# CederGroupHub/smol

Measured on AMD Instinct MI355X. Metric: attempted MC flips/s (node) + ns/flip/replica, 4096-site FCC canonical, higher is better.
Workload: dtype f64

## Files before the change

smol_amd/csrc/engine.hip:

```cpp
#include <array>
#include <map>
#include <string>
#include <thread>

#include "smolmc_common.h"

thread_local std::string smolmc_g_err;

__device__ __forceinline__ double block_sum(double v, double *sh) {
    v = wave_sum(v);
    const int lane = threadIdx.x & 63, wave = threadIdx.x >> 6, nw = blockDim.x >> 6;
    __syncthreads();
    if (lane == 0) sh[wave] = v;
    __syncthreads();
    double s = 0;
    for (int i = 0; i < nw; ++i) s += sh[i];
    return s;
}

__global__ void __launch_bounds__(256) eval_full_kernel(const RefTables T, const uint8_t *occ_all,
                                                        double *out_all, const int ce_only, const int nocc, const int M) {
    __shared__ double sh[8];
    extern __shared__ __attribute__((aligned(16))) unsigned char eval_smem[];
    const int m_eff = M > 0 ? M : 1;
// ... 635 lines not shown
            S.feat = mode.lazy() ? 0u : (uint32_t)feat;
            S.live = mode.corr_kf ? (uint32_t)t->orb_nfunc[k.orbit] : 1u;
            S.w = folded ? scale : t->ce_coefs[feat] * scale;
            S.fs = scale;
            double dmax = 0.0;
            const double *D = L.dt.data() + doff_of[key];
            for (size_t z = 0; z < L.tlen; ++z) dmax = std::max(dmax, std::fabs(D[z]));
            sum_abs += std::fabs(S.w) * dmax;
        }
        sum_abs_max = std::max(sum_abs_max, sum_abs);
    }
    L.fast_eps = 2.0 * sum_abs_max * ldexp(1.0, -19);
    return L;
}

static int commit_lean_tables(smolmc_handle *h, const smolmc_tables *t, const SiteClasses &sc, const LeanMode &mode, int NSL, int MML,
                              const Swizzle &w, std::vector<uint16_t> &lidx, const LeanDeltaTables &L) {
    LeanParams &lp = h->lp;
    memset(&lp, 0, sizeof(LeanParams));
    lp.swz_a = w.a; lp.swz_m = w.m; lp.swz_b = w.b; lp.Nlds = w.Nlds;
    lp.fast_eps = L.fast_eps;
    lp.ktab8 = (uint32_t)L.tlen * 8u;
    lp.nt8 = (uint32_t)L.NTP * 8u;
    lp.snt8 = (uint32_t)L.NTP * 8u * (uint32_t)t->max_species;
    TRY(dev_upload(h, lidx.data(), lidx.size(), &lp.idx));
    h->lean_idx_host = std::move(lidx);
    TRY(dev_upload(h, L.dt.data(), L.dt.size(), &lp.dt));
    if (mode.corr_kf) TRY(dev_upload(h, L.dtk.data(), L.dtk.size(), &lp.dtk));
    TRY(dev_upload(h, L.ls.data(), L.ls.size(), &lp.slots));
    lp.dt_len = (int)L.dt.size();
    h->lean_kf = mode.corr_kf ? SMOLMC_LEAN_MAX_KF : 0;
    h->lazy_tables = mode.lazy();
    h->lean_tables = true;
    h->lean_nslot = NSL; h->lean_mm = MML; h->lean_ncls = (int)sc.class_rep.size();
    h->site_class_host = sc.site_class;
    return 0;
}

static int build_mc_tables(smolmc_handle *h, const smolmc_tables *t) {
    const GeneralLimits lim = general_limits(t, h->Npad);
    if (lim.error) return fail(lim.error);
    if (lim.universal) return no_general(h, lim.universal);
    const SiteClasses sc = site_classes(t, lim);
    if (sc.universal) return no_general(h, sc.universal);
// ... 379 lines not shown
static int create_impl(const smolmc_tables *t, const smolmc_config *cfg, smolmc_handle **out, std::vector<int32_t> *new_of);

extern "C" void *smolmc_debug_relabel(const smolmc_tables *t, int32_t *new_of_out) {
    if (!t || validate_tables(t)) return nullptr;
    std::vector<int32_t> new_of = plan_relabelling(t);
    if (new_of.empty()) return nullptr;
    std::vector<int32_t> old_of(new_of.size());
    for (size_t p = 0; p < new_of.size(); ++p) old_of[new_of[p]] = (int32_t)p;
    RelabelledTables *rt = new RelabelledTables();
    relabel_tables(t, new_of, old_of, *rt);
    if (new_of_out) std::copy(new_of.begin(), new_of.end(), new_of_out);
    return rt;
}
extern "C" void smolmc_debug_relabel_free(void *p) { delete (RelabelledTables *)p; }

extern "C" int smolmc_create(const smolmc_tables *t, const smolmc_config *cfg, smolmc_handle **out) {
    if (!t || !cfg || !out) return fail("null argument");
    if (cfg->n_replicas <= 0) return fail("n_replicas must be positive");
    if (int rc = validate_tables(t)) return rc;
    std::vector<int32_t> new_of = plan_relabelling(t);
    if (new_of.empty()) return create_impl(t, cfg, out, nullptr);
    std::vector<int32_t> old_of(new_of.size());
    for (size_t p = 0; p < new_of.size(); ++p) old_of[new_of[p]] = (int32_t)p;
    RelabelledTables rt;
    relabel_tables(t, new_of, old_of, rt);
    return create_impl(&rt.t, cfg, out, &new_of);
}

static int wl_sum_mode_of(const smolmc_handle *h) { return (h->cfg.wl_update_period == 1 && !smolmc_env(ENV_WL_RUNNING_MEAN)) ? 1 : 0; }
static int cu_count(const smolmc_handle *h) {
// ... 319 lines not shown
    lp.tf_n = t->n_flip_vectors;
    lp.tf_sw = t->swap_weight;
    lp.tf_ln_len = ln_len;
    return 0;
}

struct LeanPlan {
    bool take = false;
    bool late = false;
    int sbase = -1, nact = 0, nc = 0;
    std::vector<double> mu_row, bias_pair, qrow, dgrow;
    bool field = false;
    bool solo = false;
    int occ = 0, wpb = 4, tf_ln_len = 0;
    size_t lds = 0, lds8 = 0;
};
static LeanPlan decide_lean(const smolmc_handle *h, const smolmc_tables *t) {
    const smolmc_config *cfg = &h->cfg;
    const KParams &kp = h->kp;
    const LeanParams &lp = h->lp;
    const bool wl = is_wl(h), table = is_table(h);
    const int wl_sum_mode = wl_sum_mode_of(h), Fk = lean_features(h, t), brows = kp.bias_rows;
    LeanPlan p;
    const bool table_wl = wl && table;
    const bool lean = h->lean_tables && Fk <= 64 &&
                (!wl || ((wl_sum_mode || (table_wl && cfg->wl_update_period < (1ll << 31))) &&
                         h->F <= 63 && cfg->wl_check_period < (1ll << 31))) &&
                (!t->has_ewald || kp.ew_compact) && t->n_sublattices == 1 && h->lean_ncls == 1 &&
                h->lean_nslot <= 4 && !smolmc_env(ENV_FORCE_GENERAL);
    if (!lean) return p;
// ... 29 lines not shown
            p.field = true;
            p.lds = with_field;
        }
    }
    if (wl && t->has_ewald && !p.field) return p;
    p.take = true;
    if (!wl && !t->has_ewald && !t->bias_type && !h->lean_kf && !table && !smolmc_env(ENV_NO_SOLO)) {
        const size_t pw = ((size_t)lp.Nlds + 64 * 8 + 15) & ~(size_t)15;
        const size_t solo_lds = pw + ((size_t)lp.dt_len + 24) * 8;
        if (solo_lds * 16 <= 160 * 1024 - 16 * 256) {
            p.solo = true;
            p.lds = solo_lds;
            if ((long)cfg->n_replicas > 16L * cu_count(h) && solo_lds * 24 <= 160 * 1024 - 24 * 256 &&
                !smolmc_env(ENV_NO_OCC6))
                p.occ = 6;
        }
    }
    if (table) {
        p.lds += 48 * 8;
        const size_t half = 80 * 1024, with_ln = p.lds + (size_t)(nact + 1) * 8;
        if (with_ln <= 150 * 1024 && (with_ln <= half || p.lds > half)) {
            p.tf_ln_len = nact + 1;
            p.lds += (size_t)(nact + 1) * 8;
        }
        const size_t per_wave = (size_t)lp.Nlds + 64 * 8 + 64 + (p.field ? (size_t)kp.ew_nact * 8 : 0);
        const size_t lds8 = p.lds + 4 * per_wave;
        if (!wl && lds8 <= 160 * 1024 && p.lds > 40 * 1024 && cfg->n_replicas % 8 == 0 &&
            (long)cfg->n_replicas >= 8L * cu_count(h)) {
            p.wpb = 8;
            p.lds8 = lds8;
// ... 14 lines not shown
    for (double v : p.mu_row) mmax = std::max(mmax, std::fabs(v));
    h->fast_eps_plain = lp.fast_eps; h->fast_eps_widenings = 1; h->mu_max_create = mmax; h->d_mu_create = lp.mu_row;
    lean_set_fast_eps(h, mmax);
    lean_fill_state(h, t, lp, 64, is_table(h) ? kp.wl_sum_mode : 1);
    lp.sbase = p.sbase; lp.nact = p.nact; lp.ncodes = p.nc;
    if (t->has_ewald) { lp.ew_act = kp.ew_act; lp.ew_qs = kp.ew_qs; lp.ew_dg = kp.ew_dg; lp.ew_frozen = kp.ew_frozen; }
    lp.ew_field = 0;
    if (p.field) {
        if (dev_upload(h, p.qrow.data(), 8, &lp.ew_qrow) || dev_upload(h, p.dgrow.data(), 8, &lp.ew_dgrow)) return 1;
        lp.ew_phi = kp.ew_phi;
        lp.ew_field = 1;
    }
    if (p.solo) {
        std::vector<uint32_t> wide(h->lean_idx_host.begin(), h->lean_idx_host.end());
        if (dev_upload(h, wide.data(), wide.size(), &lp.idx32)) return 1;
    }
    if (is_table(h) && lean_fill_table(h, t, lp, p.nc, p.nact, p.tf_ln_len)) return 1;
    h->lean_lds = p.lds;
    h->lean_solo = p.solo;
    h->lean_occ = p.occ;
    h->lean_wpb = p.wpb;
    h->lean_lds_wpb8 = p.lds8;
    return 0;
}

struct LeanMultiPlan {
    bool take = false;
    std::string reason;
    int sbase[4], nact[4], ncodes[4], cls[4];
    double cum[4], mmax = 0.0;
    std::vector<double> mu_rows, q_rows, dg_rows, bias_pairs;
    int ndims = 0, max_nact = 0, wpb = 0;
    bool phi_lds = false;
    size_t lds = 0;
};
// ... 312 lines not shown
     {"lean-multi", nullptr, nullptr, L3(multi), L3(multi_replay), L3(multi_table_replay), L3(multi_wmu)},
     {"lean-multi", nullptr, nullptr, L3(multi_bias), L3(multi_bias_replay), NONE, L3(multi_bias_wmu)},
     {"lean-multi", " wl=multi", " wl=multi-mean", L3(multi_wl), L3(multi_wl_replay), NONE, NONE},
     {"lean-multi", " wl=multi", " wl=multi-mean", L3(multi_wl_kf), NONE, NONE, NONE},
     {"lean-multi", nullptr, nullptr, L3(multi_table_bias), NONE, NONE, L3(multi_table_bias_wmu)},
     {"lean-multi", " wl=multi", " wl=multi-mean", L3(multi_table_wl), NONE, NONE, NONE},
};
#undef L2
#undef L3
#undef NONE
static_assert(sizeof(lean_families) / sizeof(lean_families[0]) == K_MULTI_TABLE_WL - K_LEAN + 1, "one row per lean family");
static LeanLauncher lean_launcher(const smolmc_handle *h, bool replay) {
    const LeanFamilyRow &row = lean_families[h->family - K_LEAN];
    const int i = h->lean_nslot == 2 ? 0 : (h->lean_nslot == 4 ? 1 : 2);
    if (!replay && h->lp.mu_stride) return row.walker_mu[i];
    return !replay ? row.run[i] : (h->cfg.step_type == SMOLMC_STEP_TABLE_FLIP ? row.table_replay[i] : row.replay[i]);
}

static KernelFamily family_of(const smolmc_handle *h, const LeanPlan &one, const LeanMultiPlan &multi) {
    const bool wl = is_wl(h), table = is_table(h), bias = h->kp.bias_type != 0;
    if (one.take)
        return bias ? (table ? K_TABLE_BIAS : K_LEAN_BIAS) : (wl && table) ? K_TABLE_WL : h->lean_kf ? K_LEAN_CORR : wl ? K_WL : K_LEAN;
    if (multi.take)
        return wl ? (h->lean_kf ? K_MULTI_WL_KF : table ? K_MULTI_TABLE_WL : K_MULTI_WL)
                  : bias ? (table ? K_MULTI_TABLE_BIAS : K_MULTI_BIAS) : K_MULTI;
    return (table || !h->general_ok) ? K_UNIVERSAL : K_GENERAL;
}

static int create_impl(const smolmc_tables *t, const smolmc_config *cfg, smolmc_handle **out, std::vector<int32_t> *new_of) {
    if (t->max_species > 255) return fail("more than 255 species codes per site");
// ... 388 lines not shown

extern "C" int smolmc_sync(smolmc_handle *h) {
    if (!h) return fail("null handle");
    HIPCHK(hipSetDevice(h->device));
    HIPCHK(hipStreamSynchronize(h->stream));
    return 0;
}

extern "C" int smolmc_kernel_info(const smolmc_handle *h, char *buf, int n) {
    if (!h || !buf || n <= 0) return fail("null argument");
    if (h->dist) return smolmc_dist_kernel_info(h, buf, n);
    const LeanFamilyRow *row = h->lean() ? &lean_families[h->family - K_LEAN] : nullptr;
    if (h->univ())
        snprintf(buf, (size_t)n, "universal occ=%s field=%d lds=%zu (%s)", h->up.occ_lds ? "lds" : "hbm", h->kp.ew_field,
                 (size_t)h->up.lds_shared + (size_t)h->up.lds_per_wave * h->univ_wpb, h->general_ok ? "TableFlip outside the lean families" : h->general_reason.c_str());
    else if (row)
        snprintf(buf, (size_t)n, "%s nslot=%d mm=%d field=%d lds=%zu%s", row->name,
                 h->lean_nslot, h->lean_mm, h->lp.ew_field, h->lean_lds,
                 h->lean_solo ? (h->lean_occ ? " solo=1 occ=6" : " solo=1") : (h->lean_kf ? " kf=1" : ""));
    else
        snprintf(buf, (size_t)n, "general nslot=%d mm=%d field=%d lds=%zu", h->nslot, h->mm, h->kp.ew_field,
                 h->lds_bytes);
    {
        const size_t used = strlen(buf);
        const bool gx = row && h->lp.ew_field && h->lp.ew_gx && used + 40 < (size_t)n;
        if (gx)
            snprintf(buf + used, (size_t)n - used, " gx=%dx%dx%dx%d", h->ew_gx_blocks, h->ew_gx_dims[0], h->ew_gx_dims[1],
                     h->ew_gx_dims[2]);
        const char *wl_tag = !row || (gx && h->family == K_WL) ? nullptr : (h->lp.wl.sum_mode ? row->wl_sums : row->wl_means);
        if (wl_tag && strlen(buf) + 24 < (size_t)n) strncat(buf, wl_tag, (size_t)n - strlen(buf) - 1);
        if (is_lazy(h) && strlen(buf) + 16 < (size_t)n) strncat(buf, " lazy-features", (size_t)n - strlen(buf) - 1);
        if (h->relabelled && strlen(buf) + 16 < (size_t)n) strncat(buf, " relabelled=1", (size_t)n - strlen(buf) - 1);
        if (!h->walker_mu.empty() && strlen(buf) + 48 < (size_t)n)
            snprintf(buf + strlen(buf), (size_t)n - strlen(buf), " walker_mu=1 mu_max=%.17g", h->mu_max);
// ... 807 lines not shown
```

smol_amd/csrc/mc_lean.h:

```cpp
#pragma once
#include "smolmc_common.h"

template <int CTRL> __device__ __forceinline__ double dpp_xor_add(double v) {
    const int lo = __builtin_amdgcn_update_dpp(__double2loint(v), __double2loint(v), CTRL, 0xf, 0xf, true);
    const int hi = __builtin_amdgcn_update_dpp(__double2hiint(v), __double2hiint(v), CTRL, 0xf, 0xf, true);
    return v + __hiloint2double(hi, lo);
}
__device__ __forceinline__ double wave_sum_all(double v) {
    v = dpp_xor_add<0xB1>(v);
    v = dpp_xor_add<0x4E>(v);
    v = dpp_xor_add<0x141>(v);
    v = dpp_xor_add<0x140>(v);
    {
        const unsigned lo = (unsigned)__double2loint(v), hi = (unsigned)__double2hiint(v);
        const auto a = __builtin_amdgcn_permlane16_swap(lo, lo, false, false);
        const auto b = __builtin_amdgcn_permlane16_swap(hi, hi, false, false);
        v = __hiloint2double((int)b[0], (int)a[0]) + __hiloint2double((int)b[1], (int)a[1]);
    }
    {
        const unsigned lo = (unsigned)__double2loint(v), hi = (unsigned)__double2hiint(v);
        const auto a = __builtin_amdgcn_permlane32_swap(lo, lo, false, false);
        const auto b = __builtin_amdgcn_permlane32_swap(hi, hi, false, false);
        v = __hiloint2double((int)b[0], (int)a[0]) + __hiloint2double((int)b[1], (int)a[1]);
    }
// ... 249 lines not shown
#define SMOLMC_LDS_F64(a) (*(const double *)(uintptr_t)(a))
#endif
template <bool ABS> __device__ __forceinline__ uint8_t occ_ld(const uint8_t *occ, uint32_t a) {
    if constexpr (ABS) return SMOLMC_LDS_U8(a);
    else return occ[a];
}
__device__ __forceinline__ uint32_t opaque_u32(uint32_t v) {
    asm volatile("" : "+s"(v));
    return v;
}
template <bool ABS> __device__ __forceinline__ void occ_st(uint8_t *occ, uint32_t a, uint8_t v) {
    if constexpr (ABS) SMOLMC_LDS_U8(a) = v;
    else occ[a] = v;
}

template <int NSLOT, int MM, int STEP, bool HAS_MU, int EWX, bool WL, bool BIAS = false, bool SOLO = false,
          int KF = 0, int OCC = 0, bool REPLAY = false>
__global__ void __attribute__((amdgpu_waves_per_eu(OCC ? OCC : 1, OCC ? OCC : 8)))
__launch_bounds__(256) mc_lean_kernel(const LeanParams P) {
    static_assert(KF == 0 || (!WL && !BIAS && !SOLO), "correlation-function tables: plain Metropolis layouts only");
    static_assert(!REPLAY || (!WL && OCC == 0), "replay: Metropolis variants (Wang-Landau: mc_wl_kernel)");
    constexpr int NACC = KF ? KF : 1;
    constexpr int EWM = EWX & 3;
    constexpr bool WMU = (EWX & 4) != 0;
    static_assert(!WMU || (HAS_MU && !WL && !REPLAY), "per-walker chemical potentials: semigrand Metropolis variants");
    constexpr bool HAS_EW = EWM != 0, ew_field = EWM == 2;
    extern __shared__ __attribute__((aligned(16))) unsigned char smem[];
    if ((uint32_t)(uintptr_t)smem != 0u) __builtin_trap();
    const int lane = threadIdx.x & 63;
    const int wave = SOLO ? 0 : threadIdx.x >> 6;
    const int nwaves = SOLO ? 1 : blockDim.x >> 6;
    const int r = uni(blockIdx.x * nwaves + wave);
    const size_t per_wave = (size_t)P.Nlds + 64 * 8 + (WL ? (size_t)P.wl.L * 24 : 0) +
                            ((HAS_EW && ew_field) ? 64 + (size_t)P.ew_nact * 8 : 0);
    double *s_dt = SOLO ? (double *)(smem + ((per_wave + 15) & ~(size_t)15)) : (double *)smem;
    const uint32_t dt_off = SOLO ? (uint32_t)((per_wave + 15) & ~(size_t)15) : 0u;
    double *s_mu = s_dt + P.dt_len;
    double *s_q = s_mu + 8, *s_dg = s_mu + 16;
    unsigned char *wbase = SOLO ? smem : (unsigned char *)(s_mu + 24) + (size_t)wave * per_wave;
    uint8_t *occ = wbase;
// ... 32 lines not shown
    if (!live) return;

    constexpr bool EPRE = HAS_EW && STEP == SMOLMC_STEP_FLIP && !REPLAY;
    uint32_t ereg[27] = {};
    bool epre_on = false;
    if (EPRE) {
        const LeanParamsKernarg Q = rare_params();
        const uint32_t *E8 = Q->ew_E8;
        epre_on = ew_field && Q->ew_gx != nullptr && (Q->ew_nact >> 6) >= 27;
        if (epre_on) {
#pragma unroll
            for (int u = 0; u < 27; ++u) ereg[u] = E8[64 * u + lane];
        }
    }

    uint32_t doff8[NSLOT], st8[NSLOT][MM], sfeat[NSLOT];
    double wgt[NSLOT], acc[NSLOT], sfs[NSLOT];
    double accK[NSLOT][NACC];
    uint32_t kslot[NSLOT];
#pragma unroll
    for (int it = 0; it < NSLOT; ++it) {
        const LeanSlot sl = P.slots[it * 64 + lane];
        doff8[it] = sl.doff8 + dt_off;
        sfeat[it] = sl.feat;
        sfs[it] = sl.live ? sl.fs : 0.0;
        kslot[it] = sl.live;
#pragma unroll
        for (int m = 0; m < MM; ++m) st8[it][m] = sl.stride8[m];
        wgt[it] = sl.w;
        acc[it] = 0.0;
#pragma unroll
        for (int k = 0; k < NACC; ++k) accK[it][k] = 0.0;
    }
    const int wl_stride = WL ? P.F : 64;
    const int wl_k = WL ? max(1, min(8, 63 / max(wl_stride, 1))) : 1;
    uint32_t sfeat_wl[NSLOT];
#pragma unroll
    for (int it = 0; it < NSLOT; ++it) sfeat_wl[it] = sfeat[it] + (uint32_t)((lane % wl_k) * wl_stride);
    int wl_rd[8];
#pragma unroll
    for (int k = 0; k < 8; ++k) wl_rd[k] = (WL && k < wl_k && lane < wl_stride) ? lane + k * wl_stride : 63;
    auto wl_cur_feat = [&]() -> double {
        const int f = lane < wl_stride ? lane : 0;
// ... 39 lines not shown
    constexpr bool FAST = !WL && !HAS_EW;
    float thr_lo = 0.0f, thr_hi = 0.0f;
    const double inv_nbeta = FAST ? 1.0 / nbeta : 0.0;
    uint32_t nacc_before = 0;
    int nsite = 0, naddr = 0;
    double *featp = P.features + (size_t)r * P.F;
    const double base_feat = lane < P.F ? featp[lane] : 0.0;
    uint32_t smp_countdown = P.smp.every ? (uint32_t)P.smp.every : 0xffffffffu;
    long long smp_index = 0;
    uint32_t W0 = 0;
    int cand[4] = {0, 0, 0, 0}, canda[4] = {0, 0, 0, 0};
    double vGc = 0.0;
    double logu = 0.0;
    unsigned long long batch64_base = ~0ull;
    unsigned long long batch_base = ~0ull;
    constexpr int ROW = NSLOT * MM;
    constexpr int NW = SOLO ? ROW : ROW / 2;
    constexpr uint32_t ENT = SOLO ? 4u : 2u;
    constexpr uint32_t SITE_BYTES = 64u * ROW * ENT;
    const __amdgpu_buffer_rsrc_t idx_rs = __builtin_amdgcn_make_buffer_rsrc(
        SOLO ? (void *)P.idx32 : (void *)P.idx, 0, 0x7fffffff, 0x00020000);
    const uint32_t lane_voff = (uint32_t)lane * (ROW * ENT);

    int s1, a1;
    RowWords<NW> row1;
    uint32_t ridx = 0;
    double lu_rp = 0.0;
    int rp_bad = 0;
    auto rp_site = [&](const uint32_t i) -> int {
        const int v = uni(P.rp_steps[((size_t)r * (uint32_t)P.steps + i) * 4]);
        return v >= 0 ? v : sbase;
    };
    {
        if (REPLAY) {
            s1 = rp_site(0u);
        } else {
            const unsigned long long sp = step - 1ull;
            const uint32_t w = (uint32_t)uni((int)philox4x32_10((uint32_t)sp, (uint32_t)(sp >> 32), 0u, 0u,
                                                                key0, key1).w[1]);
            s1 = sbase + (int)__umulhi(w, nact);
        }
        a1 = lean_swz(s1, swa, swm, swb);
        row1 = load_row<NW>(idx_rs, lane_voff, (uint32_t)s1 * SITE_BYTES);
    }

    double *wl_pend = WL ? P.wl.meanf + (size_t)r * P.wl.L * P.F : nullptr;
    double wl_pc[8] = {0.0, 0.0, 0.0, 0.0, 0.0, 0.0, 0.0, 0.0};
    auto wl_pend_sum = [&]() -> double {
        return ((wl_pc[0] + wl_pc[1]) + (wl_pc[2] + wl_pc[3])) + ((wl_pc[4] + wl_pc[5]) + (wl_pc[6] + wl_pc[7]));
    };
    uint32_t steps_left = (uint32_t)P.steps;
    while (steps_left != 0u) {
        const unsigned long long base = step & ~15ull;
        if (!REPLAY && base != batch_base) {
            batch_base = base;
            const unsigned long long st = base + (unsigned)(lane >> 2);
            const philox_out o = philox4x32_10((uint32_t)st, (uint32_t)(st >> 32), (uint32_t)(lane & 3),
                                               0u, key0, key1);
// ... 48 lines not shown
            if (u != u) u = 0.0;
            lu_rp = log(u);
            s1n = ridx + 1u < (uint32_t)P.steps ? rp_site(ridx + 1u) : s1;
            a1n = lean_swz(s1n, swa, swm, swb);
            if (FAST) {
                const double thr = lu_rp * inv_nbeta, eps = P.fast_eps + 1e-6 * fabs(thr);
                thr_lo = P.fast_eps > 0.0 ? (float)(thr - eps) : -INFINITY;
                thr_hi = P.fast_eps > 0.0 ? (float)(thr + eps) : INFINITY;
            }
        } else {
            s1n = (int)rdlane((uint32_t)nsite, l4);
            a1n = (int)rdlane((uint32_t)naddr, l4);
        }
        uint32_t va1 = (uint32_t)a1;
        asm volatile("" : "+v"(va1));
        const int o1 = uni((int)occ_ld<SOLO>(occ, va1));
        int nfl, s2, a2, n1, n2 = 0, o2 = 0;
        if (STEP != SMOLMC_STEP_SWAP) { s2 = s1; a2 = a1; }
        int fb = -1;
        if (REPLAY) {
            if (STEP == SMOLMC_STEP_FLIP) {
                nfl = rp_empty ? 0 : 1;
                n1 = rp_empty ? o1 : rq1;
                rp_bad |= (rq2 >= 0) ? 1 : 0;
            } else if (!rp_empty && rq2 >= 0) {
                nfl = 2;
                s2 = rq2;
                a2 = lean_swz(s2, swa, swm, swb);
                o2 = uni((int)occ_ld<SOLO>(occ, (uint32_t)a2));
                n2 = rq3;
                n1 = rq1;
// ... 31 lines not shown
                    if (m2) SMOLMC_CAND_TAKE(2)
                    else {
                        SMOLMC_CAND_MASK(3)
                        if (m3) SMOLMC_CAND_TAKE(3)
                        else {
                            bool hit = false;
                            const unsigned long long cur = chunk_end - chunk;
                            for (uint32_t q = 0;; ++q) {
                                const philox_out o = philox4x32_10((uint32_t)cur, (uint32_t)(cur >> 32),
                                                                   4u + 64u * q + (uint32_t)lane, 0u, key0, key1);
                                int selsite = -1, selv = 0;
#pragma unroll
                                for (int j = 3; j >= 0; --j) {
                                    const int cs = sbase + (int)__umulhi(o.w[j], nact);
                                    const int v = (int)occ[lean_swz(cs, swa, swm, swb)];
                                    if (v != o1) { selsite = cs; selv = v; }
                                }
                                const unsigned long long m = __ballot(selsite >= 0);
                                if (m) {
                                    const int b = __ffsll((long long)m) - 1;
                                    s2 = (int)rdlane((uint32_t)selsite, b);
                                    a2 = lean_swz(s2, swa, swm, swb);
                                    o2 = (int)rdlane((uint32_t)selv, b);
                                    hit = true;
                                    break;
                                }
                                if ((q & 63u) == 0) {
                                    int any = 0;
                                    for (uint32_t a = lane; a < nact; a += 64)
                                        any |= ((int)occ[lean_swz(sbase + (int)a, swa, swm, swb)] != o1);
                                    if (__ballot(any) == 0ull) break;
                                }
                            }
                            if (!hit) { nfl = 0; s2 = s1; a2 = a1; o2 = o1; }
                        }
                    }
                }
            }
#undef SMOLMC_CAND_MASK
#undef SMOLMC_CAND_TAKE
            n1 = o2;
        }

        __builtin_amdgcn_s_setprio(2);
        RowWords<NW> row2 = row1;
        if (STEP == SMOLMC_STEP_SWAP) {
            row2 = load_row<NW>(idx_rs, lane_voff, (uint32_t)s2 * SITE_BYTES);
        }
        if (WL) {
            unsafeAtomicAdd(wl_pend + lane, wl_pend_sum());
        }

        constexpr bool DIFF = STEP == SMOLMC_STEP_SWAP;
        double e = 0.0, d1[NSLOT], d2[NSLOT];
        uint32_t dp[NSLOT];
        uint32_t ad1[NSLOT], ad2[NSLOT];
        {
            const uint32_t pair1 = (uint32_t)o1 * snt8 + (uint32_t)n1 * nt8;
#pragma unroll
            for (int it = 0; it < NSLOT; ++it) {
                uint32_t a = doff8[it];
                if (DIFF) a = dp[it] = doff8[it] + pair1;
#pragma unroll
                for (int m = 0; m < MM; ++m) a += __umul24(st8[it][m], (uint32_t)occ_ld<SOLO>(occ, bounded(row_addr<SOLO, NW>(row1, it * MM + m), (uint32_t)P.Nlds)));
                if (DIFF) {
                    d1[it] = SMOLMC_LDS_F64(a);
                    if (KF) ad1[it] = a;
                } else {
                    d1[it] = SMOLMC_LDS_F64(a + pair1);
                    if (KF) ad1[it] = a + pair1;
                    e = fma(wgt[it], d1[it], e);
                }
            }
        }
        row1 = load_row<NW>(idx_rs, lane_voff, (uint32_t)s1n * SITE_BYTES);
        double ew_part = 0.0, ew_uni = 0.0;
        double dq1 = 0.0, dq2 = 0.0;
        if (HAS_EW) {
            if (ew_field) {
                dq1 = s_q[n1] - s_q[o1];
                ew_uni = 2.0 * dq1 * phi[s1 - sbase] + (s_dg[n1] - s_dg[o1]);
            } else {
                const int W = P.ew_W;
                dq1 = P.ew_qs[(size_t)s1 * W + n1] - P.ew_qs[(size_t)s1 * W + o1];
                ew_part = 2.0 * dq1 * lean_ewald_partial(P, occ, lane, s1, swa, swm, swb);
                ew_uni = 2.0 * dq1 * P.ew_frozen[s1] +
                         (P.ew_dg[(size_t)s1 * W + n1] - P.ew_dg[(size_t)s1 * W + o1]);
            }
        }
        if (STEP == SMOLMC_STEP_SWAP) {
            occ_st<SOLO>(occ, va1, (uint8_t)n1);
            const uint32_t pair2 = (uint32_t)o2 * snt8 + (uint32_t)n2 * nt8;
#pragma unroll
            for (int it = 0; it < NSLOT; ++it) {
                uint32_t a = DIFF ? dp[it] : doff8[it];
#pragma unroll
                for (int m = 0; m < MM; ++m) a += __umul24(st8[it][m], (uint32_t)occ_ld<SOLO>(occ, bounded(row_addr<SOLO, NW>(row2, it * MM + m), (uint32_t)P.Nlds)));
                if (DIFF) {
                    d1[it] -= SMOLMC_LDS_F64(a);
                    if (KF) ad2[it] = a;
                    e = fma(wgt[it], d1[it], e);
                } else {
                    d2[it] = SMOLMC_LDS_F64(a + pair2);
                    if (KF) ad2[it] = a + pair2;
                    e = fma(wgt[it], d2[it], e);
                }
            }
            if (HAS_EW) {
                if (ew_field) {
                    dq2 = s_q[n2] - s_q[o2];
                    const double cross =
                        fb >= 0 ? __hiloint2double((int)rdlane((uint32_t)__double2hiint(vGc), fb),
// ... 91 lines not shown
#pragma unroll
                for (int it = 0; it < NSLOT; ++it) acc[it] += d1[it];
                if (STEP == SMOLMC_STEP_SWAP && !DIFF) {
#pragma unroll
                    for (int it = 0; it < NSLOT; ++it) acc[it] += d2[it];
                }
            } else {
#pragma unroll
                for (int it = 0; it < NSLOT; ++it) {
                    const double dd = (STEP == SMOLMC_STEP_SWAP && !DIFF) ? d1[it] + d2[it] : d1[it];
                    __hip_atomic_fetch_add(&s_feat[sfeat_wl[it]], sfs[it] * dd, __ATOMIC_RELAXED,
                                           __HIP_MEMORY_SCOPE_WAVEFRONT);
                }
            }
            if (STEP == SMOLMC_STEP_FLIP) occ_st<SOLO>(occ, va1, (uint8_t)n1);
            if (STEP == SMOLMC_STEP_SWAP) occ_st<SOLO>(occ, (uint32_t)a2, (uint8_t)n2);
            if (HAS_EW && ew_field) {
                if (STEP == SMOLMC_STEP_SWAP) {
                    if (dq1 != 0.0 || dq2 != 0.0) field_apply2(P, phi, lane, s1, dq1, s2, dq2);
                } else if (dq1 != 0.0) {
                    field_apply<2, EPRE>(P, phi, lane, s1, dq1, ereg, epre_on);
                }
            }
            acc_mu += dMu;
            acc_ew += dEw;
            bias_acc += dB;
#pragma unroll
            for (int k = 0; k < SMOLMC_MAX_BIAS_ROWS; ++k) chg[k] += dQ[k];
            if (!FAST) H += dH;
            if (!SELACC) nacc_add++;
        };
        auto on_reject = [&]() {
            if (STEP == SMOLMC_STEP_SWAP) {
            occ_st<SOLO>(occ, va1, (uint8_t)o1);
            }
        };
        nacc_before = nacc_add;
        bool accepted = false;
        __builtin_amdgcn_s_setprio(3);
        if (FAST && !BIAS) {
            const float ef = (float)((HAS_MU && lane == 0) ? e - dMu : e);
            const float S = wave_sum_f32_uniform(ef);
            const unsigned long long bit = 1ull << (REPLAY ? 0 : l64);
            const bool ca = (__ballot(S < thr_lo) & bit) != 0ull;
            const bool cr = (__ballot(S > thr_hi) & bit) != 0ull;
            if (ca) on_accept();
            else if (cr) on_reject();
            else if (exact_decision()) on_accept();
            else on_reject();
// ... 1234 lines not shown
template <int NSLOT> static int launch_table_bias_wmu_nslot(smolmc_handle *h, const LeanParams &lp) { return launch_table_nslot<NSLOT, TV_BIAS | TV_WMU>(h, lp); }

template <int NSLOT, unsigned B> static int launch_lean_replay_kf(smolmc_handle *h, const LeanParams &lp) {
    const unsigned key = B | (lean_key(h, lp, !(B & LV_KF)) & ~(unsigned)LV_OCC6);
    return with_mm_step(h, [&](auto mm, auto step) {
        if constexpr (B & LV_KF)
            return launch_lean_variant<NSLOT, mm, step, B | LV_MU | 2, B | 2, B | LV_MU | 1, B | 1, B | LV_MU, B>(h, lp, key);
        else
            return launch_lean_variant<NSLOT, mm, step, B | LV_MU | 2, B | 2, B | LV_MU | 1, B | 1, B | LV_MU | LV_SOLO, B | LV_SOLO,
                                       B | LV_MU, B>(h, lp, key);
    });
}
template <int NSLOT> static int launch_lean_replay_nslot(smolmc_handle *h, const LeanParams &lp) {
    return h->lean_kf ? launch_lean_replay_kf<NSLOT, LV_REPLAY | LV_KF>(h, lp) : launch_lean_replay_kf<NSLOT, LV_REPLAY>(h, lp);
}
```

smol_amd/csrc/smolmc_common.h:

```cpp
#pragma once
#include <hip/hip_runtime.h>

#include <math.h>
#include <stdint.h>
#include <stdio.h>
#include <stdlib.h>
#include <string.h>

#include <algorithm>
#include <map>
#include <string>
#include <vector>

#include "../../include/smolmc.h"
#include "philox.h"

extern thread_local std::string smolmc_g_err;
static int fail(const std::string &m) {
    smolmc_g_err = m;
    return 1;
}
#define HIPCHK(x)                                                                         \
    do {                                                                                  \
        hipError_t e_ = (x);                                                              \
        if (e_ != hipSuccess)                                                             \
            return fail(std::string(#x) + ": " + hipGetErrorString(e_));                  \
    } while (0)

static const double SMOLMC_KB = 8.617333262145e-5;

enum SmolmcEnv {
    ENV_FORCE_GENERAL, ENV_FORCE_UNIVERSAL, ENV_DENSE_EWALD, ENV_LAZY_FEATURES_ONLY, ENV_NO_LAZY_FEATURES,
    ENV_NO_LEAN_ALIASED, ENV_NO_LEAN_MULTI, ENV_NO_WL_MULTI, ENV_NO_TABLE_BIAS, ENV_NO_TABLE_WL, ENV_NO_EWALD_FIELD,
    ENV_NO_EWALD_GX, ENV_NO_SOLO, ENV_NO_OCC6, ENV_NO_INKERNEL_BIAS, ENV_NO_SITE_RELABEL, ENV_MULTI_PHI_HBM,
    ENV_MULTI_PHI_LDS, ENV_UNIV_OCC_HBM, ENV_REPLAY_GENERAL, ENV_REPLAY_UNIVERSAL, ENV_WL_RUNNING_MEAN,
    ENV_WALKER_ORDER, ENV_LAUNCH_CHUNK, ENV_FAST_EPS_SCALE, ENV_NO_ROTATE, ENV_DEBUG,
    ENV_COUNT
};
struct SmolmcEnvSwitch {
    const char *name;
    bool dispatch;
    const char *purpose;
};
static constexpr SmolmcEnvSwitch smolmc_env_switches[] = {
    {"SMOLMC_FORCE_GENERAL", true, "no lean family: mc_kernel, or the universal kernel where mc_kernel cannot run"},
    {"SMOLMC_FORCE_UNIVERSAL", true, "no mc_kernel: what the lean families do not take runs on the universal kernel"},
    {"SMOLMC_DENSE_EWALD", true, "keep the dense Ewald matrix (no compact site-charge form, no potential field)"},
    {"SMOLMC_LAZY_FEATURES_ONLY", true, "several correlation functions per orbit: lazy features instead of the KF kernels"},
    {"SMOLMC_NO_LAZY_FEATURES", true, "no lazy cluster features: such models leave the lean families"},
    {"SMOLMC_NO_LEAN_ALIASED", true, "aliased supercells (a cluster holds a site twice) leave the lean families"},
    {"SMOLMC_NO_LEAN_MULTI", true, "no multi-class lean kernels (mc_lean_multi_kernel, mc_table_multi_kernel)"},
    {"SMOLMC_NO_WL_MULTI", true, "Wang-Landau leaves the multi-class lean kernels"},
    {"SMOLMC_NO_TABLE_BIAS", true, "TableFlip with an MCBias term leaves the lean table kernels"},
    {"SMOLMC_NO_TABLE_WL", true, "Wang-Landau TableFlip leaves the lean table kernels"},
    {"SMOLMC_NO_EWALD_FIELD", true, "no Ewald potential field: per-proposal row sums instead"},
    {"SMOLMC_NO_EWALD_GX", true, "no translation-compressed Ewald site kernel: the rows of G"},
    {"SMOLMC_NO_SOLO", true, "no one-wave-per-workgroup layout of mc_lean_kernel"},
    {"SMOLMC_NO_OCC6", true, "no six-waves-per-SIMD instantiation of the one-wave layout"},
    {"SMOLMC_NO_INKERNEL_BIAS", false, "biased lean walkers record their sample rows through snapshots"},
    {"SMOLMC_NO_SITE_RELABEL", true, "scattered active sites are not renumbered into one range"},
    {"SMOLMC_MULTI_PHI_HBM", true, "multi-class lean kernels: the potential field stays in HBM"},
    {"SMOLMC_MULTI_PHI_LDS", true, "multi-class lean kernels: the potential field in LDS whenever it fits"},
    {"SMOLMC_UNIV_OCC_HBM", true, "universal kernel: the occupancy stays in HBM"},
    {"SMOLMC_REPLAY_GENERAL", false, "smolmc_replay on mc_kernel where it can take the records"},
    {"SMOLMC_REPLAY_UNIVERSAL", false, "smolmc_replay on the universal kernel"},
    {"SMOLMC_WL_RUNNING_MEAN", true, "Wang-Landau keeps per-bin running means also at update_period 1"},
    {"SMOLMC_WALKER_ORDER", false, "launch-slot order of the table kernels: 0 identity, 1 (default) / 2 hot-cold pairs"},
    {"SMOLMC_LAUNCH_CHUNK", false, "lean launches split at this many steps instead of 2^30"},
    {"SMOLMC_FAST_EPS_SCALE", false, "scales the band of the float32 accept pre-test (0: every step exact)"},
    {"SMOLMC_NO_ROTATE", false, "mc_wl_kernel: no group rotation of launches beyond one round of walkers"},
    {"SMOLMC_DEBUG", false, "dispatch and replay decisions printed to stderr"},
};
static_assert(sizeof(smolmc_env_switches) / sizeof(smolmc_env_switches[0]) == ENV_COUNT, "one entry per SmolmcEnv");
// ... 484 lines not shown
    int R = 0, N = 0, Npad = 0, F = 0, Fce = 0, L = 0;
    std::vector<double> natural;
    KernelFamily family = K_GENERAL;
    bool lean() const { return family >= K_LEAN; }
    bool lean_multi() const { return family >= K_MULTI; }
    bool univ() const { return family == K_UNIVERSAL; }
    int nslot = 0, mm = 0;
    bool generic = false, idx16 = false;
    size_t lds_bytes = 0;
    int waves_per_block = 4;
    int waves_per_block_lean = 4;
    bool lean_tables = false;
    int lean_nslot = 0, lean_mm = 0, lean_ncls = 0;
    bool lean_solo = false;
    int lean_occ = 0;
    int lean_wpb = 4;
    size_t lean_lds_wpb8 = 0;
    int lean_kf = 0;
    std::vector<uint16_t> lean_idx_host;
    std::vector<int> site_class_host;
    size_t lean_lds = 0;
    LeanParams lp;
    std::vector<double> walker_mu;
    double *d_walker_mu[2] = {nullptr, nullptr};
    const double *d_mu_create = nullptr;
    double mu_max = 0.0, mu_max_create = 0.0, fast_eps_plain = 0.0;
    int fast_eps_widenings = 1;
    SampleSlot slots[2];
    int next_slot = 0;
    unsigned long long slot_seq = 0;
// ... 76 lines not shown
int smolmc_launch_general_4(smolmc_handle *h, const KParams &kp, int replay);
int smolmc_launch_general_8(smolmc_handle *h, const KParams &kp, int replay);
int smolmc_launch_general_16(smolmc_handle *h, const KParams &kp, int replay);
#define SMOLMC_LAUNCHERS2(f)                                            \
    int smolmc_launch_##f##_2(smolmc_handle *h, const LeanParams &lp); \
    int smolmc_launch_##f##_4(smolmc_handle *h, const LeanParams &lp);
#define SMOLMC_LAUNCHERS3(f) SMOLMC_LAUNCHERS2(f) int smolmc_launch_##f##_8(smolmc_handle *h, const LeanParams &lp);
SMOLMC_LAUNCHERS2(lean) SMOLMC_LAUNCHERS2(lean_replay) SMOLMC_LAUNCHERS2(table_replay)
SMOLMC_LAUNCHERS2(lean_bias) SMOLMC_LAUNCHERS2(lean_bias_replay) SMOLMC_LAUNCHERS2(lean_corr)
SMOLMC_LAUNCHERS2(wl) SMOLMC_LAUNCHERS2(wl_replay)
SMOLMC_LAUNCHERS2(table_bias) SMOLMC_LAUNCHERS2(table_wl)
SMOLMC_LAUNCHERS3(multi) SMOLMC_LAUNCHERS3(multi_replay) SMOLMC_LAUNCHERS3(multi_table_replay)
SMOLMC_LAUNCHERS3(multi_bias) SMOLMC_LAUNCHERS3(multi_bias_replay)
SMOLMC_LAUNCHERS3(multi_wl) SMOLMC_LAUNCHERS3(multi_wl_replay) SMOLMC_LAUNCHERS3(multi_wl_kf)
SMOLMC_LAUNCHERS3(multi_table_bias) SMOLMC_LAUNCHERS3(multi_table_wl)
SMOLMC_LAUNCHERS2(lean_wmu) SMOLMC_LAUNCHERS2(lean_bias_wmu) SMOLMC_LAUNCHERS2(lean_corr_wmu) SMOLMC_LAUNCHERS2(table_bias_wmu)
SMOLMC_LAUNCHERS3(multi_wmu) SMOLMC_LAUNCHERS3(multi_bias_wmu) SMOLMC_LAUNCHERS3(multi_table_bias_wmu)
#undef SMOLMC_LAUNCHERS2
#undef SMOLMC_LAUNCHERS3
#define SMOLMC_WL_ROWS 32
#define SMOLMC_WLM_LOG 16
__host__ __device__ inline size_t wl_lean_bins_bytes(int L) { return ((size_t)L + 2) * 8 + (((size_t)L * 4 + 7) & ~(size_t)7); }
__host__ __device__ inline size_t wl_multi_wave_bytes(int L, int F, int sum_mode) {
    return (size_t)L * 8 + (((size_t)L * 4 + 7) & ~(size_t)7) +
           (sum_mode ? (size_t)SMOLMC_WLM_LOG * F * 8 : (size_t)L * 8 + (size_t)SMOLMC_WL_ROWS * F * 8);
}
#define SMOLMC_LEAN_MAX_KF 6
#include "launch.h"
```

Measured before the change: 17.69 billion.

## Add solo-rows lean kernel with per-slot gather widths and address-ordered index rows

For the one-wave solo lean kernel with two slots and mm=2, this builds a host-side plan that sorts the slot lanes by how many neighbour gathers they need. Each slot then gets its own gather width, so the second slot does only one gather instead of two. The index rows are re-laid out by swizzled LDS address instead of site number, and the occupancy-store logic is adapted to match. This shortens each row and removes padded occupancy gathers per flip, at the cost of an extra kernel instantiation, a duplicate device index and slot table, and more complex swap bookkeeping. A host debug entry point is added for checking the plan.

```diff
diff --git a/smol_amd/csrc/engine.hip b/smol_amd/csrc/engine.hip
--- a/smol_amd/csrc/engine.hip
+++ b/smol_amd/csrc/engine.hip
@@ -673,6 +673,48 @@
     return L;
 }
 
+struct SoloRowsPlan {
+    int shape = 0;
+    int row_len = 0;
+    std::vector<int> perm;
+    std::vector<uint32_t> rows;
+    std::vector<LeanSlot> slots;
+};
+static SoloRowsPlan solo_rows_plan(const std::vector<uint16_t> &lidx, const LeanSlot *ls, int N, int NSL, int MML, const Swizzle &w) {
+    SoloRowsPlan p;
+    if (NSL != 2 || MML != 2 || w.Nlds < N || lidx.size() != (size_t)N * 64 * NSL * MML) return p;
+    const int NQ = 64 * NSL;
+    int nm[128];
+    for (int q = 0; q < NQ; ++q) {
+        nm[q] = 0;
+        for (int m = 0; m < MML; ++m)
+            if (ls[q].live && ls[q].stride8[m]) nm[q] = m + 1;
+    }
+    p.perm.resize(NQ);
+    for (int q = 0; q < NQ; ++q) p.perm[q] = q;
+    std::stable_sort(p.perm.begin(), p.perm.end(), [&](int a, int b) { return nm[a] > nm[b]; });
+    const int mm0 = nm[p.perm[0]], mm1 = nm[p.perm[64]];
+    if (mm0 > 2 || mm1 > 1) return p;
+    const int w0 = mm0 == 2 ? 2 : 1;
+    p.shape = w0 * 10 + 1;
+    p.row_len = w0 + 1;
+    const int RL = p.row_len, width[2] = {w0, 1}, off[2] = {0, w0};
+    p.slots.resize(NQ);
+    for (int q = 0; q < NQ; ++q) p.slots[q] = ls[p.perm[q]];
+    p.rows.resize((size_t)w.Nlds * 64 * RL);
+    for (int a = 0; a < w.Nlds; ++a)
+        for (int k = 0; k < 64 * RL; ++k) p.rows[(size_t)a * 64 * RL + k] = (uint32_t)a;
+    for (int s = 0; s < N; ++s) {
+        const int a = s ^ (((s >> w.a) & w.m) << w.b);
+        for (int q = 0; q < NQ; ++q) {
+            const int it = q / 64, ln = q % 64, oit = p.perm[q] / 64, oln = p.perm[q] % 64;
+            for (int m = 0; m < width[it]; ++m)
+                p.rows[((size_t)a * 64 + ln) * RL + off[it] + m] = lidx[(((size_t)s * 64 + oln) * NSL + oit) * MML + m];
+        }
+    }
+    return p;
+}
+
 static int commit_lean_tables(smolmc_handle *h, const smolmc_tables *t, const SiteClasses &sc, const LeanMode &mode, int NSL, int MML,
                               const Swizzle &w, std::vector<uint16_t> &lidx, const LeanDeltaTables &L) {
     LeanParams &lp = h->lp;
@@ -687,6 +729,7 @@
     TRY(dev_upload(h, L.dt.data(), L.dt.size(), &lp.dt));
     if (mode.corr_kf) TRY(dev_upload(h, L.dtk.data(), L.dtk.size(), &lp.dtk));
     TRY(dev_upload(h, L.ls.data(), L.ls.size(), &lp.slots));
+    h->lean_slots_host = L.ls;
     lp.dt_len = (int)L.dt.size();
     h->lean_kf = mode.corr_kf ? SMOLMC_LEAN_MAX_KF : 0;
     h->lazy_tables = mode.lazy();
@@ -1096,6 +1139,50 @@
 }
 extern "C" void smolmc_debug_relabel_free(void *p) { delete (RelabelledTables *)p; }
 
+struct SoloRowsDebug {
+    int shape, row_len, N, Nlds, swz_a, swz_m, swz_b, nslot, mm;
+    const int *perm;
+    const uint32_t *rows;
+    const LeanSlot *slots;
+    const uint16_t *lean_rows;
+    const LeanSlot *lean_slots;
+    SoloRowsPlan plan;
+    std::vector<uint16_t> lidx;
+    std::vector<LeanSlot> ls;
+};
+static void build_mc_tables_host(const smolmc_tables *t, const smolmc_config *cfg, SoloRowsDebug &d) {
+    smolmc_handle h;
+    h.cfg = *cfg;
+    h.Npad = (t->num_sites + 15) / 16 * 16;
+    d.N = t->num_sites;
+    const GeneralLimits lim = general_limits(t, h.Npad);
+    if (lim.error || lim.universal) return;
+    const SiteClasses sc = site_classes(t, lim);
+    if (sc.universal) return;
+    const LeanMode mode = lean_mode(&h, t, lim, sc);
+    if (*mode.reason || mode.corr_kf) return;
+    const int NSL = sc.niter_max <= 2 ? 2 : (sc.niter_max <= 4 ? 4 : 8), MML = sc.lean_need_mm <= 2 ? 2 : 3;
+    d.nslot = NSL; d.mm = MML;
+    d.lidx = lean_index_rows(t, sc, NSL, MML);
+    const Swizzle w = choose_swizzle(d.lidx, sc, t->num_sites, h.Npad, NSL * MML);
+    for (uint16_t &x : d.lidx) x = (uint16_t)(x ^ (((x >> w.a) & w.m) << w.b));
+    d.Nlds = w.Nlds; d.swz_a = w.a; d.swz_m = w.m; d.swz_b = w.b;
+    const LeanDeltaTables L = lean_delta_tables(t, sc, mode, NSL, MML);
+    if (L.too_large) return;
+    d.ls = L.ls;
+    if (sc.class_rep.size() == 1) d.plan = solo_rows_plan(d.lidx, d.ls.data(), t->num_sites, NSL, MML, w);
+}
+extern "C" void *smolmc_debug_solo_rows(const smolmc_tables *t, const smolmc_config *cfg) {
+    if (!t || !cfg || validate_tables(t)) return nullptr;
+    SoloRowsDebug *d = new SoloRowsDebug();
+    build_mc_tables_host(t, cfg, *d);
+    d->shape = d->plan.shape; d->row_len = d->plan.row_len;
+    d->perm = d->plan.perm.data(); d->rows = d->plan.rows.data(); d->slots = d->plan.slots.data();
+    d->lean_rows = d->lidx.data(); d->lean_slots = d->ls.data();
+    return d;
+}
+extern "C" void smolmc_debug_solo_rows_free(void *p) { delete (SoloRowsDebug *)p; }
+
 extern "C" int smolmc_create(const smolmc_tables *t, const smolmc_config *cfg, smolmc_handle **out) {
     if (!t || !cfg || !out) return fail("null argument");
     if (cfg->n_replicas <= 0) return fail("n_replicas must be positive");
@@ -1445,6 +1532,7 @@
     bool solo = false;
     int occ = 0, wpb = 4, tf_ln_len = 0;
     size_t lds = 0, lds8 = 0;
+    SoloRowsPlan rows;
 };
 static LeanPlan decide_lean(const smolmc_handle *h, const smolmc_tables *t) {
     const smolmc_config *cfg = &h->cfg;
@@ -1504,6 +1592,9 @@
             if ((long)cfg->n_replicas > 16L * cu_count(h) && solo_lds * 24 <= 160 * 1024 - 24 * 256 &&
                 !smolmc_env(ENV_NO_OCC6))
                 p.occ = 6;
+            if (!smolmc_env(ENV_NO_SOLO_ROWS))
+                p.rows = solo_rows_plan(h->lean_idx_host, h->lean_slots_host.data(), t->num_sites, h->lean_nslot, h->lean_mm,
+                                        Swizzle{lp.swz_a, lp.swz_m, lp.swz_b, lp.Nlds});
         }
     }
     if (table) {
@@ -1548,11 +1639,15 @@
     if (p.solo) {
         std::vector<uint32_t> wide(h->lean_idx_host.begin(), h->lean_idx_host.end());
         if (dev_upload(h, wide.data(), wide.size(), &lp.idx32)) return 1;
+        if (p.rows.shape && (dev_upload(h, p.rows.rows.data(), p.rows.rows.size(), &h->d_rows_idx32) ||
+                             dev_upload(h, p.rows.slots.data(), p.rows.slots.size(), &h->d_rows_slots)))
+            return 1;
     }
     if (is_table(h) && lean_fill_table(h, t, lp, p.nc, p.nact, p.tf_ln_len)) return 1;
     h->lean_lds = p.lds;
     h->lean_solo = p.solo;
     h->lean_occ = p.occ;
+    h->solo_rows = p.solo ? p.rows.shape : 0;
     h->lean_wpb = p.wpb;
     h->lean_lds_wpb8 = p.lds8;
     return 0;
@@ -1895,6 +1990,7 @@
     const LeanFamilyRow &row = lean_families[h->family - K_LEAN];
     const int i = h->lean_nslot == 2 ? 0 : (h->lean_nslot == 4 ? 1 : 2);
     if (!replay && h->lp.mu_stride) return row.walker_mu[i];
+    if (!replay && h->family == K_LEAN && h->solo_rows && h->lean_nslot == 2) return smolmc_launch_lean_rows_2;
     return !replay ? row.run[i] : (h->cfg.step_type == SMOLMC_STEP_TABLE_FLIP ? row.table_replay[i] : row.replay[i]);
 }
 
@@ -2313,10 +2409,13 @@
     if (h->univ())
         snprintf(buf, (size_t)n, "universal occ=%s field=%d lds=%zu (%s)", h->up.occ_lds ? "lds" : "hbm", h->kp.ew_field,
                  (size_t)h->up.lds_shared + (size_t)h->up.lds_per_wave * h->univ_wpb, h->general_ok ? "TableFlip outside the lean families" : h->general_reason.c_str());
-    else if (row)
+    else if (row) {
         snprintf(buf, (size_t)n, "%s nslot=%d mm=%d field=%d lds=%zu%s", row->name,
                  h->lean_nslot, h->lean_mm, h->lp.ew_field, h->lean_lds,
                  h->lean_solo ? (h->lean_occ ? " solo=1 occ=6" : " solo=1") : (h->lean_kf ? " kf=1" : ""));
+        if (h->family == K_LEAN && h->solo_rows && !h->lp.mu_stride && strlen(buf) + 12 < (size_t)n)
+            snprintf(buf + strlen(buf), (size_t)n - strlen(buf), " rows=%d", h->solo_rows);
+    }
     else
         snprintf(buf, (size_t)n, "general nslot=%d mm=%d field=%d lds=%zu", h->nslot, h->mm, h->kp.ew_field,
                  h->lds_bytes);
diff --git a/smol_amd/csrc/lean_rows_n2.hip b/smol_amd/csrc/lean_rows_n2.hip
--- /dev/null
+++ b/smol_amd/csrc/lean_rows_n2.hip
@@ -0,0 +1,5 @@
+#include "mc_lean.h"
+
+int smolmc_launch_lean_rows_2(smolmc_handle *h, const LeanParams &lp) {
+    return launch_lean_rows_nslot<2>(h, lp);
+}
diff --git a/smol_amd/csrc/mc_lean.h b/smol_amd/csrc/mc_lean.h
--- a/smol_amd/csrc/mc_lean.h
+++ b/smol_amd/csrc/mc_lean.h
@@ -287,6 +287,12 @@
     else occ[a] = v;
 }
 
+constexpr bool lean_rows(int MM) { return MM >= 10; }
+constexpr int lean_mm_of(int MM, int it) { return !lean_rows(MM) ? MM : (it == 0 ? MM / 10 : MM % 10); }
+constexpr int lean_mm_max(int MM) { return !lean_rows(MM) ? MM : (MM / 10 > MM % 10 ? MM / 10 : MM % 10); }
+constexpr int lean_row_off(int MM, int it) { return !lean_rows(MM) ? it * MM : (it == 0 ? 0 : MM / 10); }
+constexpr int lean_row_len(int MM, int NSLOT) { return !lean_rows(MM) ? NSLOT * MM : MM / 10 + MM % 10; }
+
 template <int NSLOT, int MM, int STEP, bool HAS_MU, int EWX, bool WL, bool BIAS = false, bool SOLO = false,
           int KF = 0, int OCC = 0, bool REPLAY = false>
 __global__ void __attribute__((amdgpu_waves_per_eu(OCC ? OCC : 1, OCC ? OCC : 8)))
@@ -297,6 +303,9 @@
     constexpr int EWM = EWX & 3;
     constexpr bool WMU = (EWX & 4) != 0;
     static_assert(!WMU || (HAS_MU && !WL && !REPLAY), "per-walker chemical potentials: semigrand Metropolis variants");
+    constexpr bool ROWS = lean_rows(MM);
+    constexpr int MMX = lean_mm_max(MM);
+    static_assert(!ROWS || (SOLO && NSLOT == 2 && EWX == 0 && !REPLAY && KF == 0 && !WL && !BIAS), "solo rows: plain Metropolis, solo layout");
     constexpr bool HAS_EW = EWM != 0, ew_field = EWM == 2;
     extern __shared__ __attribute__((aligned(16))) unsigned char smem[];
     if ((uint32_t)(uintptr_t)smem != 0u) __builtin_trap();
@@ -359,7 +368,7 @@
         }
     }
 
-    uint32_t doff8[NSLOT], st8[NSLOT][MM], sfeat[NSLOT];
+    uint32_t doff8[NSLOT], st8[NSLOT][MMX], sfeat[NSLOT];
     double wgt[NSLOT], acc[NSLOT], sfs[NSLOT];
     double accK[NSLOT][NACC];
     uint32_t kslot[NSLOT];
@@ -371,7 +380,7 @@
         sfs[it] = sl.live ? sl.fs : 0.0;
         kslot[it] = sl.live;
 #pragma unroll
-        for (int m = 0; m < MM; ++m) st8[it][m] = sl.stride8[m];
+        for (int m = 0; m < (ROWS ? lean_mm_of(MM, it) : MM); ++m) st8[it][m] = sl.stride8[m];
         wgt[it] = sl.w;
         acc[it] = 0.0;
 #pragma unroll
@@ -441,7 +450,7 @@
     double logu = 0.0;
     unsigned long long batch64_base = ~0ull;
     unsigned long long batch_base = ~0ull;
-    constexpr int ROW = NSLOT * MM;
+    constexpr int ROW = lean_row_len(MM, NSLOT);
     constexpr int NW = SOLO ? ROW : ROW / 2;
     constexpr uint32_t ENT = SOLO ? 4u : 2u;
     constexpr uint32_t SITE_BYTES = 64u * ROW * ENT;
@@ -468,7 +477,7 @@
             s1 = sbase + (int)__umulhi(w, nact);
         }
         a1 = lean_swz(s1, swa, swm, swb);
-        row1 = load_row<NW>(idx_rs, lane_voff, (uint32_t)s1 * SITE_BYTES);
+        row1 = load_row<NW>(idx_rs, lane_voff, (uint32_t)(ROWS ? a1 : s1) * SITE_BYTES);
     }
 
     double *wl_pend = WL ? P.wl.meanf + (size_t)r * P.wl.L * P.F : nullptr;
@@ -547,7 +556,8 @@
         }
         uint32_t va1 = (uint32_t)a1;
         asm volatile("" : "+v"(va1));
-        const int o1 = uni((int)occ_ld<SOLO>(occ, va1));
+        const int vo1 = (int)occ_ld<SOLO>(occ, va1);
+        const int o1 = uni(vo1);
         int nfl, s2, a2, n1, n2 = 0, o2 = 0;
         if (STEP != SMOLMC_STEP_SWAP) { s2 = s1; a2 = a1; }
         int fb = -1;
@@ -609,13 +619,13 @@
                                 for (int j = 3; j >= 0; --j) {
                                     const int cs = sbase + (int)__umulhi(o.w[j], nact);
                                     const int v = (int)occ[lean_swz(cs, swa, swm, swb)];
-                                    if (v != o1) { selsite = cs; selv = v; }
+                                    if (v != o1) { selsite = ROWS ? lean_swz(cs, swa, swm, swb) : cs; selv = v; }
                                 }
                                 const unsigned long long m = __ballot(selsite >= 0);
                                 if (m) {
                                     const int b = __ffsll((long long)m) - 1;
                                     s2 = (int)rdlane((uint32_t)selsite, b);
-                                    a2 = lean_swz(s2, swa, swm, swb);
+                                    a2 = ROWS ? s2 : lean_swz(s2, swa, swm, swb);
                                     o2 = (int)rdlane((uint32_t)selv, b);
                                     hit = true;
                                     break;
@@ -640,7 +650,7 @@
         __builtin_amdgcn_s_setprio(2);
         RowWords<NW> row2 = row1;
         if (STEP == SMOLMC_STEP_SWAP) {
-            row2 = load_row<NW>(idx_rs, lane_voff, (uint32_t)s2 * SITE_BYTES);
+            row2 = load_row<NW>(idx_rs, lane_voff, (uint32_t)(ROWS ? a2 : s2) * SITE_BYTES);
         }
         if (WL) {
             unsafeAtomicAdd(wl_pend + lane, wl_pend_sum());
@@ -657,7 +667,7 @@
                 uint32_t a = doff8[it];
                 if (DIFF) a = dp[it] = doff8[it] + pair1;
 #pragma unroll
-                for (int m = 0; m < MM; ++m) a += __umul24(st8[it][m], (uint32_t)occ_ld<SOLO>(occ, bounded(row_addr<SOLO, NW>(row1, it * MM + m), (uint32_t)P.Nlds)));
+                for (int m = 0; m < (ROWS ? lean_mm_of(MM, it) : MM); ++m) a += __umul24(st8[it][m], (uint32_t)occ_ld<SOLO>(occ, bounded(row_addr<SOLO, NW>(row1, (ROWS ? lean_row_off(MM, it) : it * MM) + m), (uint32_t)P.Nlds)));
                 if (DIFF) {
                     d1[it] = SMOLMC_LDS_F64(a);
                     if (KF) ad1[it] = a;
@@ -668,7 +678,7 @@
                 }
             }
         }
-        row1 = load_row<NW>(idx_rs, lane_voff, (uint32_t)s1n * SITE_BYTES);
+        row1 = load_row<NW>(idx_rs, lane_voff, (uint32_t)(ROWS ? a1n : s1n) * SITE_BYTES);
         double ew_part = 0.0, ew_uni = 0.0;
         double dq1 = 0.0, dq2 = 0.0;
         if (HAS_EW) {
@@ -690,7 +700,7 @@
             for (int it = 0; it < NSLOT; ++it) {
                 uint32_t a = DIFF ? dp[it] : doff8[it];
 #pragma unroll
-                for (int m = 0; m < MM; ++m) a += __umul24(st8[it][m], (uint32_t)occ_ld<SOLO>(occ, bounded(row_addr<SOLO, NW>(row2, it * MM + m), (uint32_t)P.Nlds)));
+                for (int m = 0; m < (ROWS ? lean_mm_of(MM, it) : MM); ++m) a += __umul24(st8[it][m], (uint32_t)occ_ld<SOLO>(occ, bounded(row_addr<SOLO, NW>(row2, (ROWS ? lean_row_off(MM, it) : it * MM) + m), (uint32_t)P.Nlds)));
                 if (DIFF) {
                     d1[it] -= SMOLMC_LDS_F64(a);
                     if (KF) ad2[it] = a;
@@ -812,7 +822,7 @@
                 }
             }
             if (STEP == SMOLMC_STEP_FLIP) occ_st<SOLO>(occ, va1, (uint8_t)n1);
-            if (STEP == SMOLMC_STEP_SWAP) occ_st<SOLO>(occ, (uint32_t)a2, (uint8_t)n2);
+            if (STEP == SMOLMC_STEP_SWAP) occ_st<SOLO>(occ, (uint32_t)a2, (uint8_t)(ROWS ? vo1 : n2));
             if (HAS_EW && ew_field) {
                 if (STEP == SMOLMC_STEP_SWAP) {
                     if (dq1 != 0.0 || dq2 != 0.0) field_apply2(P, phi, lane, s1, dq1, s2, dq2);
@@ -830,7 +840,7 @@
         };
         auto on_reject = [&]() {
             if (STEP == SMOLMC_STEP_SWAP) {
-            occ_st<SOLO>(occ, va1, (uint8_t)o1);
+            occ_st<SOLO>(occ, va1, (uint8_t)(ROWS ? vo1 : o1));
             }
         };
         nacc_before = nacc_add;
@@ -2095,3 +2105,15 @@
 template <int NSLOT> static int launch_lean_replay_nslot(smolmc_handle *h, const LeanParams &lp) {
     return h->lean_kf ? launch_lean_replay_kf<NSLOT, LV_REPLAY | LV_KF>(h, lp) : launch_lean_replay_kf<NSLOT, LV_REPLAY>(h, lp);
 }
+
+template <int NSLOT> static int launch_lean_rows_nslot(smolmc_handle *h, const LeanParams &lp) {
+    LeanParams q = lp;
+    q.idx32 = h->d_rows_idx32;
+    q.slots = h->d_rows_slots;
+    const unsigned key = lean_key(h, q, true);
+    return first_match<21, 11>(h->solo_rows, [&](auto mm) {
+        return first_match<SMOLMC_STEP_SWAP, SMOLMC_STEP_FLIP>(h->cfg.step_type, [&](auto step) {
+            return launch_lean_variant<NSLOT, mm, step, LV_SOLO, LV_MU | LV_SOLO, LV_SOLO | LV_OCC6, LV_MU | LV_SOLO | LV_OCC6>(h, q, key);
+        });
+    });
+}
diff --git a/smol_amd/csrc/smolmc_common.h b/smol_amd/csrc/smolmc_common.h
--- a/smol_amd/csrc/smolmc_common.h
+++ b/smol_amd/csrc/smolmc_common.h
@@ -32,7 +32,7 @@
 enum SmolmcEnv {
     ENV_FORCE_GENERAL, ENV_FORCE_UNIVERSAL, ENV_DENSE_EWALD, ENV_LAZY_FEATURES_ONLY, ENV_NO_LAZY_FEATURES,
     ENV_NO_LEAN_ALIASED, ENV_NO_LEAN_MULTI, ENV_NO_WL_MULTI, ENV_NO_TABLE_BIAS, ENV_NO_TABLE_WL, ENV_NO_EWALD_FIELD,
-    ENV_NO_EWALD_GX, ENV_NO_SOLO, ENV_NO_OCC6, ENV_NO_INKERNEL_BIAS, ENV_NO_SITE_RELABEL, ENV_MULTI_PHI_HBM,
+    ENV_NO_EWALD_GX, ENV_NO_SOLO, ENV_NO_OCC6, ENV_NO_SOLO_ROWS, ENV_NO_INKERNEL_BIAS, ENV_NO_SITE_RELABEL, ENV_MULTI_PHI_HBM,
     ENV_MULTI_PHI_LDS, ENV_UNIV_OCC_HBM, ENV_REPLAY_GENERAL, ENV_REPLAY_UNIVERSAL, ENV_WL_RUNNING_MEAN,
     ENV_WALKER_ORDER, ENV_LAUNCH_CHUNK, ENV_FAST_EPS_SCALE, ENV_NO_ROTATE, ENV_DEBUG,
     ENV_COUNT
@@ -57,6 +57,7 @@
     {"SMOLMC_NO_EWALD_GX", true, "no translation-compressed Ewald site kernel: the rows of G"},
     {"SMOLMC_NO_SOLO", true, "no one-wave-per-workgroup layout of mc_lean_kernel"},
     {"SMOLMC_NO_OCC6", true, "no six-waves-per-SIMD instantiation of the one-wave layout"},
+    {"SMOLMC_NO_SOLO_ROWS", true, "one-wave layout: no per-slot gather widths / address-ordered index rows (lean_rows_n2.hip)"},
     {"SMOLMC_NO_INKERNEL_BIAS", false, "biased lean walkers record their sample rows through snapshots"},
     {"SMOLMC_NO_SITE_RELABEL", true, "scattered active sites are not renumbered into one range"},
     {"SMOLMC_MULTI_PHI_HBM", true, "multi-class lean kernels: the potential field stays in HBM"},
@@ -571,6 +572,10 @@
     int lean_nslot = 0, lean_mm = 0, lean_ncls = 0;
     bool lean_solo = false;
     int lean_occ = 0;
+    int solo_rows = 0;
+    const uint32_t *d_rows_idx32 = nullptr;
+    const LeanSlot *d_rows_slots = nullptr;
+    std::vector<LeanSlot> lean_slots_host;
     int lean_wpb = 4;
     size_t lean_lds_wpb8 = 0;
     int lean_kf = 0;
@@ -677,6 +682,7 @@
 SMOLMC_LAUNCHERS3(multi_bias) SMOLMC_LAUNCHERS3(multi_bias_replay)
 SMOLMC_LAUNCHERS3(multi_wl) SMOLMC_LAUNCHERS3(multi_wl_replay) SMOLMC_LAUNCHERS3(multi_wl_kf)
 SMOLMC_LAUNCHERS3(multi_table_bias) SMOLMC_LAUNCHERS3(multi_table_wl)
+int smolmc_launch_lean_rows_2(smolmc_handle *h, const LeanParams &lp);
 SMOLMC_LAUNCHERS2(lean_wmu) SMOLMC_LAUNCHERS2(lean_bias_wmu) SMOLMC_LAUNCHERS2(lean_corr_wmu) SMOLMC_LAUNCHERS2(table_bias_wmu)
 SMOLMC_LAUNCHERS3(multi_wmu) SMOLMC_LAUNCHERS3(multi_bias_wmu) SMOLMC_LAUNCHERS3(multi_table_bias_wmu)
 #undef SMOLMC_LAUNCHERS2
```

Measured after the change: 18.51 billion, median of 6. 1.05x the previous value.
